# wangruichens/recsys

Hardware: AMD Instinct MI355X
Metric: examples/sec (higher is better)
Workload: dtype f32; 1 GPU; deepfm.py Criteo-39 d=16 DNN 100-100 bs=256/replica, full train step (fwd+bwd+TF1 Adam), adam_mode=tf1_dense, hip_graph=True, steps_per_graph=16; global_batch=256, parallelism=dp1, adam_window=8, reported=median repeat

## Files before the change

include/rsx.h:

```cpp
#ifndef RSX_H_
#define RSX_H_
#include <stddef.h>
#include <stdint.h>

#ifdef __cplusplus
extern "C" {
#endif

typedef void* rsx_stream_t;

typedef enum {
  RSX_OK = 0,
  RSX_EINVAL = -1,
  RSX_ELAUNCH = -2,
  RSX_EUNSUPPORTED = -3,
  RSX_EDATA = -4,
  RSX_ECOMM = -5
} rsx_status;

int rsx_version(void);
unsigned long long rsx_dbg_launch_count(void);
const char* rsx_strerror(int status);


// ... 32 lines not shown
                           float* E, float* S, float* y1, float* y2, uint64_t w1_field_mask, int B, int F, int D,
                           const rsx_sort_job* sort_h, rsx_stream_t stream);

typedef struct {
  const int32_t* segid;
  float* P;
  float* P1;
  float* G;
  float* gw1;
  const int32_t* row_off;
  int32_t null_row;
  uint64_t skip_mask;
} rsx_seg_partials;
#define RSX_NULL_NONE (-1)
#define RSX_NULL_LAST_ROW (-2)
typedef struct {
  int32_t examples;
  int64_t stride_floats;
} rsx_example_blocks;
int rsx_segsum_partials(const float* tables, const float* S, const float* dX, const float* gy1, const float* gy2,
                        const int32_t* perm, const int32_t* seg_off, const int32_t* uniq_row,
                        const rsx_seg_partials* ws_h, uint64_t w1_field_mask, int B, int F, int D, int stride,
                        int null_row, const rsx_example_blocks* blocks_h, rsx_stream_t stream);


int rsx_segsum_bwd(const float* tables, const float* S, const float* dX, const float* gy1, const float* gy2,
                   const int32_t* perm, const int32_t* seg_off, const int32_t* uniq_row, const int32_t* nuniq,
                   float* G, float* gw1, uint64_t w1_field_mask, int B, int F, int D, int stride,
                   const rsx_seg_partials* partials_h, const rsx_example_blocks* blocks_h, rsx_stream_t stream);

typedef enum {
  RSX_ADAM_DENSE = 0,
  RSX_ADAM_TABLE_TF1 = 1,
  RSX_ADAM_VEC_SLOT = 2,
  RSX_ADAM_TABLE_ROWS = 3,
  RSX_ADAM_VEC_ROWS = 4,
  RSX_ADAM_TABLE_TF1_COLD = 5,
  RSX_ADAM_VEC_COLD = 6,
  RSX_ADAM_VEC_ROWS_DENSE = 7
} rsx_adam_kind;

typedef struct {
  int32_t kind;
  int32_t d;
  int64_t n;
  float* var;
  float* m;
  float* v;
  float* g;
  const int32_t* slot;
  const int32_t* uniq_row;
  const int32_t* nuniq;
  int32_t B;
  int32_t stride;
  int32_t zero_grad;
  const int32_t* slot_w[7];
  int32_t g_replicas;
  int64_t g_replica_stride;
} rsx_adam_seg;

#define RSX_ADAM_MAX_SEGS 12
#define RSX_ADAM_STATE_WORDS (4 + 32 * 32)
int rsx_adam_state_init_h(float* state_h , float beta1, float beta2);
int rsx_adam_tf1_multi(const rsx_adam_seg* segs_h, int nseg, float* state, float lr, float beta1,
                       float beta2, float eps, rsx_stream_t stream);

#define RSX_OPT_ADAGRAD 1
#define RSX_OPT_FTRL 2
typedef struct {
  int32_t kind;
  float lr, lr_power, l1, l2, l2_shrinkage;
} rsx_sparse_opt_hp;
int rsx_sparse_opt_multi(const rsx_adam_seg* segs_h, int nseg, float* state, const rsx_sparse_opt_hp* hp,
                         rsx_stream_t stream);

typedef struct {
  const rsx_adam_seg* segs;
  int32_t nseg;
  float lr, beta1, beta2, eps;
  float* state;
  uint32_t blk_lo, blk_hi;
  int32_t window_block_u;
  int32_t alphas_from_state;
} rsx_adam_slice;
int64_t rsx_adam_num_blocks(const rsx_adam_seg* segs_h, int nseg);
int64_t rsx_adam_num_blocks_u(const rsx_adam_seg* segs_h, int nseg, int window_block_u);
typedef struct rsx_table_set {
  float* tables; float* m; float* v;
  const float* dX;
  const rsx_seg_partials* partials;
} rsx_table_set;
#define RSX_ADAM_WINDOW_MAX 8
typedef struct {
  int32_t k;
  int32_t cur;
  int32_t max_unique;
  const int32_t* uniq_row[RSX_ADAM_WINDOW_MAX];
  const int32_t* nuniq[RSX_ADAM_WINDOW_MAX];
  const int32_t* slot[RSX_ADAM_WINDOW_MAX];
} rsx_adam_window;
int rsx_segsum_adam_rows(float* tables, float* m_t, float* v_t, float* w1, float* m_w, float* v_w, const float* S,
                         const float* dX, const float* gy1, const float* gy2, const int32_t* perm, const int32_t* seg_off,
                         const int32_t* uniq_row, const int32_t* nuniq, uint64_t w1_field_mask, int B, int F, int D,
                         int stride, const rsx_adam_seg* extra_segs_h, int n_extra, const rsx_adam_slice* sweep_h,
                         const rsx_seg_partials* partials_h, const rsx_example_blocks* blocks_h,
                         const rsx_table_set* second_h, const rsx_adam_window* win_h, float* state, int advance_step,
                         float lr, float beta1, float beta2, float eps, rsx_stream_t stream);
int rsx_segsum_adam_rows2(float* tables, float* m_t, float* v_t, float* w1, float* m_w, float* v_w, const float* S,
                          const float* dX, const float* gy1, const float* gy2, const int32_t* perm, const int32_t* seg_off,
                          const int32_t* uniq_row, const int32_t* nuniq, uint64_t w1_field_mask, int B, int F, int D,
                          int stride, const rsx_adam_seg* extra_segs_h, int n_extra, const rsx_adam_slice* sweep_h,
                          const rsx_seg_partials* partials_h, const rsx_example_blocks* blocks_h,
                          const rsx_table_set* second_h, const rsx_adam_window* win_h, float* state, int advance_step,
                          float lr, float beta1, float beta2, float eps, int w1_stride, int w1_sparse_formula,
                          rsx_stream_t stream);

#define RSX_UNIQ_MAX_RANKS 8
#define RSX_UNIQ_MAX_PARTS 64
int rsx_segsum_bwd_packed(const float* tables, const float* S, const float* dX, const float* gy1, const float* gy2,
                          const int32_t* perm, const int32_t* seg_off, const int32_t* uniq_row, const int32_t* nuniq,
                          float* G, float* gw1, uint64_t w1_field_mask, int B, int F, int D, int stride, int null_row,
                          const rsx_seg_partials* partials_h, const int32_t* goff, rsx_stream_t stream);
typedef struct {
  const int32_t* uniq_row;
  const int32_t* nuniq;
  int32_t* keys;
} rsx_uniq_pack_job;
int rsx_uniq_pack(const rsx_uniq_pack_job* jobs_h, int njobs, const int32_t* goff, const int32_t* row_off, int F, int stride,
                  int parts, int max_cap , rsx_stream_t stream);
typedef struct {
  int32_t* uniq_row;
  int32_t* nuniq;
  int32_t* slot;
  int32_t* src;
} rsx_uniq_merge_job;
int rsx_uniq_merge(const int32_t* keys, long long rank_stride, int job_stride, const rsx_uniq_merge_job* jobs_h, int njobs,
                   const int32_t* goff, const int32_t* row_off, int32_t* part_counts, int parts, int max_rows_per_field,
                   int max_entries, int F, int N, int stride, rsx_stream_t stream);
int rsx_merged_adam_rows(float* tables, float* m_t, float* v_t, float* w1, float* m_w, float* v_w, const float* G,
                         const float* gw1, long long rank_stride, int N, const int32_t* src, const int32_t* goff,
                         const int32_t* uniq_row, const int32_t* nuniq, uint64_t w1_field_mask, int max_units, int F, int D,
                         int stride, const rsx_adam_seg* extra_segs_h, int n_extra, const rsx_adam_slice* sweep_h,
                         const rsx_table_set* second_h, const rsx_adam_window* win_h, float* state, int advance_step,
                         float lr, float beta1, float beta2, float eps, int w1_stride, int w1_sparse_formula,
                         rsx_stream_t stream);
#define RSX_COMM_UNIQUE_ID_BYTES 128
typedef void* rsx_comm_t;
int rsx_comm_available_h(int* version_out );
const char* rsx_comm_last_error_h(void);
int rsx_comm_unique_id_h(void* id_out );
int rsx_comm_init_h(const void* unique_id, int rank, int world, rsx_comm_t* comm_out);
int rsx_comm_destroy_h(rsx_comm_t comm);
int rsx_comm_rank_world_h(rsx_comm_t comm, int* rank, int* world);
int rsx_all_gather(rsx_comm_t comm, const void* send, void* recv, size_t bytes_per_rank, rsx_stream_t stream);
int rsx_all_reduce_sum_f32(rsx_comm_t comm, const float* send, float* recv, size_t n, rsx_stream_t stream);
int rsx_all_reduce_all_gather(rsx_comm_t comm, float* grad, size_t n, const void* send, void* recv, size_t bytes_per_rank,
                              rsx_stream_t stream);

int rsx_copy_bytes(void* dst, const void* src, size_t nbytes, rsx_stream_t stream);
int rsx_adam_slice_run(const rsx_adam_slice* slice_h, rsx_stream_t stream);
int rsx_adam_fast_math_selftest(unsigned long long* counts, uint32_t seed, int div_iters, int exhaustive_div,
                                rsx_stream_t stream);

#define RSX_TOWER_FIXED_STATS_MIN_B 513
#define RSX_TOWER_FIXED_STATS_DOUBLES(N) (8 * 4 * (((N) + 15) / 16 * 16))
int rsx_tower_fwd_layer(const float* in, const float* W, const float* bias, float* a_out, double* fstat_out,
// ... 531 lines not shown
```

recsys_amd/_lib.py:

```python
import contextlib
import ctypes as C
import gc
import os

_HERE = os.path.dirname(os.path.abspath(__file__))
LIB_PATH = os.environ.get("RSX_LIB_PATH") or os.path.join(_HERE, "librsx.so")

(RSX_ADAM_DENSE, RSX_ADAM_TABLE_TF1, RSX_ADAM_VEC_SLOT, RSX_ADAM_TABLE_ROWS, RSX_ADAM_VEC_ROWS, RSX_ADAM_TABLE_TF1_COLD,
 RSX_ADAM_VEC_COLD, RSX_ADAM_VEC_ROWS_DENSE) = range(8)
RSX_ADAM_MAX_SEGS = 12
RSX_OPT_ADAGRAD, RSX_OPT_FTRL = 1, 2


class RsxError(RuntimeError):
    pass



FORMS = {
    "scatter_riders": ("1", "reductions only the optimizer reads ride in the scatter's stage-A launch (0: launches of their own)"),
    "sort_in_gather": ("0", "deepfm.py: the dedup sort rides in the gather launch instead of the first tower-forward launch"),
    "sort_ride_max": ("2048", "largest global batch whose dedup sort rides in another launch"),
    "din_side_sort": ("1", "din.py: the ids-only branch (sort + sweep) on a side stream of the step's graph"),
    "din_side_sort_dp": ("1", "the same under data parallelism"),
    "din_gather_ride": ("1", "din.py: the history gather rides in the prepare launch"),
    "mlp_reduce_ride": ("1", "din.py: the fused MLP's gradient reduce rides in the pooling backward launch"),
    "mlp_fuse": ("1", "a batch-norm-free tower as ONE launch (csrc/mlp_fused.hip) instead of 2L + 2"),
    "fm_fuse": ("1", "fm.py: forward + head in one launch"),
    "fuse_gather": ("1", "the input_layer lookup rides in the first tower-forward launch"),
    "gather_cross": ("1", "dcn.py: lookup + cross forward as one launch"),
    "cross_ride": ("1", "dcn.py: the cross layers' backward rides in the last tower layer's backward launch (0: a launch of its own)"),
    "win_separate_sorts": ("0", "debugging aid: an optimizer window's k sorts as k launches"),
    "cin_dx_fsplit": ("1", "xdeepfm.py: the first CIN layer's data gradients split their fields over two workgroups per tile"),
    "cin_wide": ("1", "xdeepfm.py --cin_bf16: the wide-tile kernels"),
    "cin_gather_ride": ("1", "xdeepfm.py: the lookup rides in the filter-preparation launch"),
    "cin_dx0_ride": ("1", "xdeepfm.py: the dX0 tile reduce rides in the weight-gradient launch"),
    "xdfm_sort_ride": ("1", "xdeepfm.py: the dedup sort rides in a tower launch"),
    "dp_eager_tail": ("1", "segmented data-parallel graphs: the step's train_op as an eager tail"),
    "dp_prefetch": ("0", "segmented data-parallel graphs: the next step's ids all-gather issued early"),
    "window_stage": ("", "'memcpy': staged windows fetched with hipMemcpyAsync instead of the copy kernel"),
    "window_sets": ("2", "captured instances of a streaming window that take turns"),
    "input_thread": ("0", "the input iterator on a thread of its own"),
    "launch_thread": ("0", "streaming windows issued by a thread of their own"),
    "adam_window_large": ("4", "steps per optimizer window above the small-batch threshold"),
}


def form(name):
    name = name.lower()
    default = FORMS[name][0]
    spec = os.environ.get("RSX_FORMS")
    if spec:
        for item in spec.split(","):
            k, _, v = item.partition("=")
            k = k.strip().lower()
            if k and k not in FORMS:
                raise RsxError("RSX_FORMS: unknown launch form %r (known: %s)" % (k, ", ".join(sorted(FORMS))))
            if k == name:
                return v.strip()
    return default


class AdamSeg(C.Structure):
    _fields_ = [("kind", C.c_int32), ("d", C.c_int32), ("n", C.c_int64),
                ("var", C.c_void_p), ("m", C.c_void_p), ("v", C.c_void_p), ("g", C.c_void_p),
                ("slot", C.c_void_p), ("uniq_row", C.c_void_p), ("nuniq", C.c_void_p),
                ("B", C.c_int32), ("stride", C.c_int32), ("zero_grad", C.c_int32), ("slot_w", C.c_void_p * 7),
                ("g_replicas", C.c_int32), ("g_replica_stride", C.c_int64)]


class AdamSlice(C.Structure):
    _fields_ = [("segs", C.POINTER(AdamSeg)), ("nseg", C.c_int32), ("lr", C.c_float), ("beta1", C.c_float),
                ("beta2", C.c_float), ("eps", C.c_float), ("state", C.c_void_p), ("blk_lo", C.c_uint32),
                ("blk_hi", C.c_uint32), ("window_block_u", C.c_int32), ("alphas_from_state", C.c_int32)]


class ExampleBlocks(C.Structure):
    _fields_ = [("examples", C.c_int32), ("stride_floats", C.c_int64)]


class SegPartials(C.Structure):
    _fields_ = [("segid", C.c_void_p), ("P", C.c_void_p), ("P1", C.c_void_p), ("G", C.c_void_p), ("gw1", C.c_void_p),
                ("row_off", C.c_void_p), ("null_row", C.c_int32), ("skip_mask", C.c_uint64)]

    def __init__(self, segid=None, P=None, P1=None, G=None, gw1=None, row_off=None, null_row=-1, skip_mask=0):
        super().__init__(segid, P, P1, G, gw1, row_off, null_row, skip_mask)


NULL_NONE, NULL_LAST_ROW = -1, -2


class MlpStep(C.Structure):
    _fields_ = [("X", C.c_void_p), ("W", C.c_void_p * 3), ("b", C.c_void_p * 3), ("masks", C.c_void_p * 3),
                ("wout", C.c_void_p), ("bout", C.c_void_p), ("s0", C.c_void_p), ("labels", C.c_void_p),
                ("rng_step", C.c_void_p), ("prob", C.c_void_p), ("dX", C.c_void_p), ("gs0", C.c_void_p),
                ("workspace", C.c_void_p), ("dW", C.c_void_p * 3), ("db", C.c_void_p * 3), ("dwout", C.c_void_p),
                ("dbout", C.c_void_p), ("loss", C.c_void_p), ("seed", C.c_uint32), ("dropout_rate", C.c_float),
                ("loss_scale", C.c_float), ("B", C.c_int32), ("K0", C.c_int32), ("L", C.c_int32), ("widths", C.c_int32 * 3),
                ("defer_reduce", C.c_int32), ("reserved", C.c_int32)]


class MlpReduceJob(C.Structure):
    _fields_ = [("part", C.c_void_p), ("poff", C.c_longlong * 4), ("dW", C.c_void_p * 3), ("db", C.c_void_p * 3),
                ("dwout", C.c_void_p), ("dbout", C.c_void_p), ("loss", C.c_void_p), ("K", C.c_int32 * 3), ("N", C.c_int32 * 3),
                ("e4_end", C.c_uint32 * 3), ("e4_last", C.c_uint32), ("L", C.c_int32), ("nwg", C.c_int32), ("NPo", C.c_int32),
                ("NL", C.c_int32), ("inv_B", C.c_double)]


class DwReduceJob(C.Structure):
    _fields_ = [("partials", C.c_void_p), ("dW", C.c_void_p), ("db", C.c_void_p), ("sb", C.c_int32), ("K", C.c_int32),
                ("N", C.c_int32), ("layout", C.c_int32)]


class CrossReduceJob(C.Structure):
    _fields_ = [("part", C.c_void_p), ("dW", C.c_void_p), ("dB", C.c_void_p), ("dwout", C.c_void_p), ("RT", C.c_int32),
                ("n", C.c_int32), ("L", C.c_int32), ("dim", C.c_int32)]


class TowerBwdExtra(C.Structure):
    _fields_ = [("accumulate_dx", C.c_int32), ("x0", C.c_void_p), ("cW", C.c_void_p), ("cB", C.c_void_p), ("s", C.c_void_p),
                ("gz", C.c_void_p), ("wout", C.c_void_p), ("dX", C.c_void_p), ("dcW", C.c_void_p), ("dcB", C.c_void_p),
                ("dwout", C.c_void_p), ("workspace", C.c_void_p), ("dim", C.c_int32), ("L", C.c_int32),
                ("reduce_out", C.POINTER(CrossReduceJob))]


class VecReduceJob(C.Structure):
    _fields_ = [("part", C.c_void_p), ("out", C.c_void_p), ("G", C.c_int32), ("n", C.c_int32)]


class ScatterRiders(C.Structure):
    _fields_ = [("dw", DwReduceJob * 4), ("n_dw", C.c_int32), ("n_vec", C.c_int32), ("cross", CrossReduceJob),
                ("vec", VecReduceJob * 2)]


class GatherJob(C.Structure):
    _fields_ = [("table", C.c_void_p), ("ids", C.c_void_p), ("out", C.c_void_p), ("n", C.c_int64), ("K", C.c_int32),
                ("ld_out", C.c_int32), ("row_base", C.c_int32), ("ld_table", C.c_int32)]


class TableSet(C.Structure):
    _fields_ = [("tables", C.c_void_p), ("m", C.c_void_p), ("v", C.c_void_p), ("dX", C.c_void_p), ("partials", C.c_void_p)]


class CinDwJob(C.Structure):
    _fields_ = [("Xk", C.c_void_p), ("ws", C.c_void_p), ("dW", C.c_void_p), ("dc", C.c_void_p), ("H", C.c_int32), ("N", C.c_int32),
                ("dc_rows", C.c_int32)]


class GatherTwoJob(C.Structure):
    _fields_ = [("tables1", C.c_void_p), ("w1", C.c_void_p), ("tables2", C.c_void_p), ("row_off", C.c_void_p), ("ids", C.c_void_p),
                ("num_x", C.c_void_p), ("num_w", C.c_void_p), ("E1", C.c_void_p), ("E2", C.c_void_p), ("y1", C.c_void_p),
                ("w1_field_mask", C.c_uint64), ("B", C.c_int32), ("F", C.c_int32), ("D", C.c_int32), ("ND", C.c_int32)]


class UniqPackJob(C.Structure):
    _fields_ = [("uniq_row", C.c_void_p), ("nuniq", C.c_void_p), ("keys", C.c_void_p)]

# ... 295 lines not shown
```

recsys_amd/csrc/adam.hip:

```cpp
#include "adam_device.h"

__global__ __launch_bounds__(ADAM_T) void adam_multi_k(const AdamArgs a) {
  const float b1p = a.state[0], b2p = a.state[1];
  adam_block(a, blockIdx.x);
  __syncthreads();
  if (threadIdx.x == 0 && adam_arrive_last(a.state, a.total_blocks)) {
    a.state[0] = b1p * a.b1;
    a.state[1] = b2p * a.b2;
    reinterpret_cast<uint32_t*>(a.state)[3] += 1u;
  }
}

extern "C" int rsx_adam_state_init_h(float* state_h, float beta1, float beta2) {
  if (!state_h) return RSX_EINVAL;
  state_h[0] = beta1;
  state_h[1] = beta2;
  reinterpret_cast<uint32_t*>(state_h)[2] = 0u;
  reinterpret_cast<uint32_t*>(state_h)[3] = 1u;
  return RSX_OK;
}

extern "C" int rsx_adam_tf1_multi(const rsx_adam_seg* segs_h, int nseg, float* state, float lr, float beta1,
                                  float beta2, float eps, rsx_stream_t stream) {
  AdamArgs a;
  uint32_t blocks = 0;
  const int rc = adam_build_args(segs_h, nseg, state, lr, beta1, beta2, eps, a, &blocks);
  if (rc != RSX_OK) return rc;
  if (blocks == 0) return RSX_OK;
  RSX_LAUNCH(adam_multi_k, dim3(blocks), dim3(ADAM_T), 0, rsx_s(stream), a);
  RSX_CHECK_LAUNCH();
  return RSX_OK;
}

extern "C" int64_t rsx_adam_num_blocks(const rsx_adam_seg* segs_h, int nseg) {
  return rsx_adam_num_blocks_u(segs_h, nseg, 0);
}
extern "C" int64_t rsx_adam_num_blocks_u(const rsx_adam_seg* segs_h, int nseg, int window_block_u) {
  AdamArgs a;
  uint32_t blocks = 0;
  float dummy;
  const int rc = adam_build_args(segs_h, nseg, &dummy, 0.f, 0.f, 0.f, 0.f, a, &blocks, window_block_u);
  return rc != RSX_OK ? (int64_t)rc : (int64_t)blocks;
}

__global__ __launch_bounds__(ADAM_T) void adam_slice_k(const AdamSlice s) { adam_block(s.args, s.blk_lo + blockIdx.x); }

#ifndef RSX_ADAM_WIN_OCC
#define RSX_ADAM_WIN_OCC 3
#endif
template <int NW>
__global__ __launch_bounds__(ADAM_T, RSX_ADAM_WIN_OCC) void adam_window_k(const AdamSlice s) {
  if (blockIdx.x == 0 && threadIdx.x == 0 && s.blk_lo == 0 && !s.args.alpha_src) adam_publish_step_sizes<NW>(s.args);
  adam_window_block<NW>(s.args, s.blk_lo + blockIdx.x);
}
template <int NW>
static void launch_window(const AdamSlice& s, hipStream_t st) {
  RSX_LAUNCH(adam_window_k<NW>, dim3(s.n_blk), dim3(ADAM_T), 0, st, s);
}

extern "C" int rsx_adam_slice_run(const rsx_adam_slice* slice_h, rsx_stream_t stream) {
  AdamSlice s;
  const int rc = adam_build_slice(slice_h, s);
  if (rc != RSX_OK) return rc;
  if (s.n_blk == 0) return RSX_OK;
  if (s.args.win_u != 0) return RSX_EUNSUPPORTED;
  const dim3 grid(s.n_blk), block(ADAM_T);
  switch (s.args.nw) {
    case 0: RSX_LAUNCH(adam_slice_k, grid, block, 0, rsx_s(stream), s); break;
    case 1: launch_window<1>(s, rsx_s(stream)); break;
    case 2: launch_window<2>(s, rsx_s(stream)); break;
    case 3: launch_window<3>(s, rsx_s(stream)); break;
    case 4: launch_window<4>(s, rsx_s(stream)); break;
    case 5: launch_window<5>(s, rsx_s(stream)); break;
    case 6: launch_window<6>(s, rsx_s(stream)); break;
    default: launch_window<7>(s, rsx_s(stream)); break;
  }
  RSX_CHECK_LAUNCH();
  return RSX_OK;
}

namespace {
__device__ __forceinline__ uint32_t st_mix(uint32_t x) {
  x ^= x >> 16; x *= 0x7feb352du; x ^= x >> 15; x *= 0x846ca68bu; x ^= x >> 16;
  return x;
}
__global__ void st_sqrt_k(const uint32_t lo, const uint32_t hi, unsigned long long* bad) {
  const uint32_t n = hi - lo;
  unsigned long long mine = 0;
  for (uint64_t i = ((uint64_t)blockIdx.x * blockDim.x + threadIdx.x) * 2u; i < n; i += (uint64_t)gridDim.x * blockDim.x * 2u) {
    const uint32_t b0 = lo + (uint32_t)i, b1 = i + 1 < n ? b0 + 1 : b0;
    const float x0 = __uint_as_float(b0), x1 = __uint_as_float(b1);
    const rsx_f2 s = rsx_sqrt2_fast((rsx_f2){x0, x1});
    mine += __float_as_uint(s.x) != __float_as_uint(sqrtf(x0));
    mine += b1 != b0 && __float_as_uint(s.y) != __float_as_uint(sqrtf(x1));
  }
  if (mine) atomicAdd(bad, mine);
}
__global__ void st_div_k(const uint32_t seed, const int iters, unsigned long long* bad) {
  uint32_t s = st_mix(seed ^ (blockIdx.x * blockDim.x + threadIdx.x) * 0x9e3779b9u);
  unsigned long long mine = 0;
  for (int it = 0; it < iters; ++it) {
    float n[2], d[2];
    for (int k = 0; k < 2; ++k) {
      s = st_mix(s + 0x632be5abu);
      const uint32_t en = 127 - 94 + s % (94 + 34 + 1);
      s = st_mix(s + 1);
      const uint32_t ed = 127 - 30 + s % (30 + 21 + 1);
      s = st_mix(s + 2);
      uint32_t mn = s & 0x7fffffu;
      const uint32_t sg = s >> 31;
      if ((s >> 23 & 31u) == 0u) mn = (s >> 28) & 1u ? 0x7fffffu : 0u;
      if (en == 127u + 34u) mn = 0u;
      s = st_mix(s + 3);
      uint32_t md = s & 0x7fffffu;
      if ((s >> 23 & 15u) == 0u) md = (s >> 27) & 1u ? 0x7fffffu : 0u;
      if (ed == 127u + 21u) md = 0u;
      n[k] = __uint_as_float((sg << 31) | (en << 23) | mn);
      if ((s >> 28) == 0u) n[k] = 0.f;
      d[k] = __uint_as_float((ed << 23) | md);
    }
    const rsx_f2 q = rsx_div2_fast((rsx_f2){n[0], n[1]}, (rsx_f2){d[0], d[1]});
    mine += __float_as_uint(q.x) != __float_as_uint(n[0] / d[0]);
    mine += __float_as_uint(q.y) != __float_as_uint(n[1] / d[1]);
  }
  if (mine) atomicAdd(bad, mine);
}

__global__ void st_div_all_k(const uint32_t md_lo, unsigned long long* bad) {
  unsigned long long mine = 0;
  const float d = __uint_as_float(0x3f800000u | (md_lo + blockIdx.x));
  for (uint32_t mn = threadIdx.x * 2u; mn < (1u << 23); mn += blockDim.x * 2u) {
    const float n0 = __uint_as_float(0x3f800000u | mn), n1 = __uint_as_float(0x3f800000u | (mn + 1u));
    const rsx_f2 q = rsx_div2_fast((rsx_f2){n0, n1}, (rsx_f2){d, d});
    mine += __float_as_uint(q.x) != __float_as_uint(n0 / d);
    mine += __float_as_uint(q.y) != __float_as_uint(n1 / d);
  }
  if (mine) atomicAdd(bad, mine);
}
}

extern "C" int rsx_adam_fast_math_selftest(unsigned long long* counts, uint32_t seed, int div_iters, int exhaustive_div,
                                           rsx_stream_t stream) {
  if (!counts || div_iters < 0) return RSX_EINVAL;
  hipStream_t st = rsx_s(stream);
  if (hipMemsetAsync(counts, 0, 4 * sizeof(unsigned long long), st) != hipSuccess) return RSX_ELAUNCH;
  RSX_LAUNCH(st_sqrt_k, dim3(4096), dim3(256), 0, st, (127u - 96u) << 23, (127u + 41u) << 23, counts);
  const int grid = 4096, block = 256;
  if (div_iters > 0) RSX_LAUNCH(st_div_k, dim3(grid), dim3(block), 0, st, seed, div_iters, counts + 1);
  const unsigned long long pairs = 2ull * grid * block * (unsigned long long)div_iters;
  if (hipMemcpyAsync(counts + 2, &pairs, sizeof(pairs), hipMemcpyHostToDevice, st) != hipSuccess) return RSX_ELAUNCH;
  if (exhaustive_div) {
    for (uint32_t lo = 0; lo < (1u << 23); lo += (1u << 18)) {
      RSX_LAUNCH(st_div_all_k, dim3(1u << 18), dim3(256), 0, st, lo, counts + 3);
      if (hipStreamSynchronize(st) != hipSuccess) return RSX_ELAUNCH;
    }
  }
  if (hipStreamSynchronize(st) != hipSuccess) return RSX_ELAUNCH;
  RSX_CHECK_LAUNCH();
// ... 3 lines not shown
```

recsys_amd/csrc/adam_device.h:

```cpp
#pragma once
#include "adam_fast.h"
#include "rsx_common.h"

struct SegDev {
  int32_t kind, d;
  long long n;
  float *var, *m, *v, *g;
  const int32_t *slot, *uniq_row, *nuniq;
  int32_t B, stride, zero_grad;
  uint32_t blk_begin;
  int32_t g_rep, g_rep_stride4;
};
constexpr int ADAM_WMAX = RSX_ADAM_WINDOW_MAX - 1;
struct AdamArgs {
  SegDev seg[RSX_ADAM_MAX_SEGS];
  const int32_t* slot_w0;
  long long slot_w_stride;
  int32_t nw;
  int32_t nseg;
  float lr, b1, b2, eps;
  float* state;
  uint32_t total_blocks;
  int32_t win_u, alpha_src;
};
// ... 273 lines not shown
        const int f = (int)(sidx / s.B), j = (int)(sidx - (long long)f * s.B);
        if (j < s.nuniq[f]) {
          const long long sl = (long long)f * s.stride + j;
          const int r = s.uniq_row[sl];
          float g = s.g[sl];
          for (int rr = 1; rr < s.g_rep; ++rr) g += s.g[(long long)rr * 4 * s.g_rep_stride4 + sl];
          if (s.kind == RSX_ADAM_VEC_ROWS_DENSE) adam_dense1(s.var[r], s.m[r], s.v[r], g, h);
          else adam_sparse1(s.var[r], s.m[r], s.v[r], g, true, h);
        }
      }
    }
  }
}

#ifndef RSX_ADAM_WIN_FAST
#define RSX_ADAM_WIN_FAST 1
#endif

__device__ __forceinline__ float rsx_sqrt1_fast(const float x) {
  const float r = __builtin_amdgcn_rsqf(x), g = x * r, hh = r * 0.5f;
  return __builtin_fmaf(__builtin_fmaf(-g, g, x), hh, g);
}
__device__ __forceinline__ float rsx_div1_fast(const float n, const float d) {
  float r = __builtin_amdgcn_rcpf(d);
  r = __builtin_fmaf(__builtin_fmaf(-d, r, 1.f), r, r);
  const float q = n * r;
  return __builtin_fmaf(__builtin_fmaf(-d, q, n), r, q);
}
template <bool DENSE>
__device__ __forceinline__ void adam_zero_grad1(float& var, float& m, float& v, const bool active, const Hp& h) {
  float m1, v1, n;
  if constexpr (DENSE) {
    m1 = m + (0.f - m) * h.omb1;
    v1 = v + (0.f * 0.f - v) * h.omb2;
    n = m1 * h.alpha;
  } else {
    m1 = m * h.b1;
    v1 = v * h.b2;
    n = h.alpha * m1;
  }
  const bool vz = __float_as_uint(v1) == 0u && __float_as_uint(n) == 0u;
  const float d = (vz ? 0.f : rsx_sqrt1_fast(vz ? 1.f : v1)) + h.eps;
  const uint32_t vb = __float_as_uint(v1), nb = __float_as_uint(n), na = nb & 0x7fffffffu, db = __float_as_uint(d);
  constexpr uint32_t V_LO = (127u - 96u) << 23, V_HI = (127u + 41u) << 23;
  constexpr uint32_t D_LO = (127u - 30u) << 23, D_HI = (127u + 21u) << 23;
  constexpr uint32_t N_LO = (127u - 94u) << 23, N_HI = (127u + 34u) << 23;
  const bool ok = (vz || (vb - V_LO) < (V_HI - V_LO)) && (db - D_LO) <= (D_HI - D_LO) &&
                  (nb == 0u || (na - N_LO) <= (N_HI - N_LO));
  if (RSX_ADAM_WIN_FAST && __builtin_amdgcn_ballot_w64(active && !ok) == 0ull) {
    if (active) {
      var = var - rsx_div1_fast(n, d);
      m = m1;
      v = v1;
    }
  } else if (active) {
    if constexpr (DENSE) adam_dense1(var, m, v, 0.f, h);
    else adam_sparse1(var, m, v, 0.f, false, h);
  }
}


__device__ __forceinline__ void adam_zero_grad2(rsx_f2& var, rsx_f2& m, rsx_f2& v, const float alpha, const Hp& h) {
  m = m * h.b1;
  v = v * h.b2;
  const rsx_f2 n = m * alpha;
  const rsx_f2 d = rsx_sqrt2_fast(v) + h.eps;
  var = var - rsx_div2_fast(n, d);
}
__device__ __forceinline__ bool adam_win_guard1(const float var, const float m, const float v, const uint32_t m_lo_bits) {
  const uint32_t vb = __float_as_uint(v), mb = __float_as_uint(m), ma = mb & 0x7fffffffu;
  const uint32_t va = __float_as_uint(var) & 0x7fffffffu;
  constexpr uint32_t V_LO = (127u - 86u) << 23, V_HI = (127u + 40u) << 23, M_HI = (127u + 30u) << 23;
  constexpr uint32_t VAR_LO = (127u - 24u) << 23;
  const bool v_ok = (vb - V_LO) <= (V_HI - V_LO);
  const bool m_mid = (ma - m_lo_bits) <= (M_HI - m_lo_bits);
  const bool m_tiny = ma < m_lo_bits && va >= VAR_LO;
  return !(mb == 0u ? (v_ok || vb == 0u) : (v_ok && (m_mid || m_tiny)));
}
__device__ __forceinline__ bool adam_win_guard4(const float4& var, const float4& m, const float4& v, const uint32_t m_lo_bits) {
  return adam_win_guard1(var.x, m.x, v.x, m_lo_bits) | adam_win_guard1(var.y, m.y, v.y, m_lo_bits) |
         adam_win_guard1(var.z, m.z, v.z, m_lo_bits) | adam_win_guard1(var.w, m.w, v.w, m_lo_bits);
}

template <int NW, int U = ADAM_U>
__device__ __forceinline__ void adam_window_block(const AdamArgs& a, const uint32_t blk, const int tid = threadIdx.x) {
  constexpr int nw = NW;
  constexpr int HB = RSX_ADAM_WIN_HB;
  constexpr int NB = U / HB;
  static_assert(U % HB == 0 && U <= ADAM_U, "U");
  int si = 0;
#pragma unroll 1
  for (int k = 1; k < a.nseg; ++k)
    if (blk >= a.seg[k].blk_begin) si = k;
  const SegDev& s = a.seg[si];
  if (s.kind != RSX_ADAM_TABLE_TF1_COLD) {
    adam_block(a, blk, tid);
    return;
  }
  Hp h;
  h.b1 = a.b1;
  h.b2 = a.b2;
  h.omb1 = 1.0f - a.b1;
  h.omb2 = 1.0f - a.b2;
  h.eps = a.eps;
  AlphaW aw;
  adam_step_sizes(a, nw, h.alpha, aw);
  float amin = h.alpha, amax = h.alpha;
#pragma unroll
  for (int j = 0; j < NW; ++j) {
    amin = fminf(amin, aw.get(j));
    amax = fmaxf(amax, aw.get(j));
  }
  const bool fast_ok = RSX_ADAM_WIN_FAST && a.b1 >= 0.85f && a.b1 < 1.f && a.b2 >= 0.5f && a.b2 < 1.f && a.eps >= 0x1p-30f &&
                       a.eps <= 1.f && amin >= 0x1p-24f && amax <= 16.f && amax <= 4.f * amin;
  const uint32_t m_lo_bits = __float_as_uint(fast_ok ? 0x1p-90f / amin : 1.f);
  const int32_t* __restrict__ swb = a.slot_w0;
  const int sws = (int)a.slot_w_stride;
  float4* __restrict__ var4 = reinterpret_cast<float4*>(s.var);
  float4* __restrict__ m4 = reinterpret_cast<float4*>(s.m);
  float4* __restrict__ v4 = reinterpret_cast<float4*>(s.v);
  const long long base = (long long)(blk - s.blk_begin) * ((long long)ADAM_T * U);
  const int lpr = s.d >> 2;
  const long long n4 = s.n * lpr;
  const bool pow2 = (lpr & (lpr - 1)) == 0;
  const int lsh = 31 - __clz(lpr);
  struct Batch {
    float4 var[HB], m[HB], v[HB];
    long long ec[HB];
    int t[HB];
    bool live[HB];
  };
  auto issue = [&](const int b, Batch& B) {
#pragma unroll
    for (int u = 0; u < HB; ++u) {
      const long long e = base + (long long)(b * HB + u) * ADAM_T + tid;
      B.ec[u] = e < n4 ? e : n4 - 1;
      B.live[u] = e < n4;
      const long long row = pow2 ? (B.ec[u] >> lsh) : (B.ec[u] / lpr);
      B.t[u] = s.slot[row];
#pragma unroll
      for (int l = 0; l < NW; ++l) B.t[u] &= swb[l * sws + (int)row];
    }
#pragma unroll
    for (int u = 0; u < HB; ++u) {
#if RSX_ADAM_NT
      B.var[u] = __builtin_nontemporal_load(&var4[B.ec[u]]);
      B.m[u] = __builtin_nontemporal_load(&m4[B.ec[u]]);
      B.v[u] = __builtin_nontemporal_load(&v4[B.ec[u]]);
#else
      B.var[u] = var4[B.ec[u]];
      B.m[u] = m4[B.ec[u]];
      B.v[u] = v4[B.ec[u]];
#endif
    }
  };
  auto store = [&](const Batch& B) {
#pragma unroll
    for (int u = 0; u < HB; ++u) {
      if (B.live[u] && B.t[u] < 0) {
#if RSX_ADAM_NT
        __builtin_nontemporal_store(B.var[u], &var4[B.ec[u]]);
        __builtin_nontemporal_store(B.m[u], &m4[B.ec[u]]);
        __builtin_nontemporal_store(B.v[u], &v4[B.ec[u]]);
#else
        var4[B.ec[u]] = B.var[u];
        m4[B.ec[u]] = B.m[u];
        v4[B.ec[u]] = B.v[u];
#endif
      }
    }
  };
  uint32_t redo = fast_ok ? 0u : (1u << NB) - 1u;
  auto finish = [&](const int b, Batch& B) {
    if (!fast_ok) return;
    bool bad = false;
#pragma unroll
    for (int u = 0; u < HB; ++u) bad |= adam_win_guard4(B.var[u], B.m[u], B.v[u], m_lo_bits);
    if (__builtin_amdgcn_ballot_w64(bad) != 0ull) {
      redo |= 1u << b;
      return;
    }
    rsx_f2 var2[HB][2], m2[HB][2], v2[HB][2];
#pragma unroll
    for (int u = 0; u < HB; ++u) {
      var2[u][0] = (rsx_f2){B.var[u].x, B.var[u].y}; var2[u][1] = (rsx_f2){B.var[u].z, B.var[u].w};
      m2[u][0] = (rsx_f2){B.m[u].x, B.m[u].y}; m2[u][1] = (rsx_f2){B.m[u].z, B.m[u].w};
      v2[u][0] = (rsx_f2){B.v[u].x == 0.f ? 1.f : B.v[u].x, B.v[u].y == 0.f ? 1.f : B.v[u].y};
      v2[u][1] = (rsx_f2){B.v[u].z == 0.f ? 1.f : B.v[u].z, B.v[u].w == 0.f ? 1.f : B.v[u].w};
    }
    auto step = [&](const float alpha) {
#pragma unroll
      for (int u = 0; u < HB; ++u) {
        adam_zero_grad2(var2[u][0], m2[u][0], v2[u][0], alpha, h);
        adam_zero_grad2(var2[u][1], m2[u][1], v2[u][1], alpha, h);
      }
    };
    step(h.alpha);
#pragma unroll 1
    for (int j = 0; j < NW; ++j) step(aw.get(j));
#pragma unroll
    for (int u = 0; u < HB; ++u) {
      B.var[u] = make_float4(var2[u][0].x, var2[u][0].y, var2[u][1].x, var2[u][1].y);
      B.m[u] = make_float4(m2[u][0].x, m2[u][0].y, m2[u][1].x, m2[u][1].y);
      B.v[u] = make_float4(B.v[u].x == 0.f ? 0.f : v2[u][0].x, B.v[u].y == 0.f ? 0.f : v2[u][0].y,
                           B.v[u].z == 0.f ? 0.f : v2[u][1].x, B.v[u].w == 0.f ? 0.f : v2[u][1].y);
    }
    store(B);
  };
  {
    Batch bt[2];
    issue(0, bt[0]);
#pragma unroll
    for (int b = 0; b < NB; ++b) {
      if (b + 1 < NB) issue(b + 1, bt[(b + 1) & 1]);
      finish(b, bt[b & 1]);
    }
  }
  redo = __builtin_amdgcn_readfirstlane(redo);
  if (redo != 0u) {
#pragma unroll 1
    for (int b = 0; b < NB; ++b) {
      if (!(redo >> b & 1u)) continue;
      Batch B;
      issue(b, B);
#pragma unroll
      for (int u = 0; u < HB; ++u) {
        F4_APPLY(adam_sparse1, B.var[u], B.m[u], B.v[u], F4Z, false, h);
#pragma unroll 1
        for (int j = 0; j < NW; ++j) {
          Hp hj = h;
          hj.alpha = aw.get(j);
          F4_APPLY(adam_sparse1, B.var[u], B.m[u], B.v[u], F4Z, false, hj);
        }
      }
      store(B);
    }
  }
}

static inline int adam_build_args(const rsx_adam_seg* segs_h, int nseg, float* state, float lr, float beta1, float beta2,
                                  float eps, AdamArgs& a, uint32_t* blocks_out, int win_u = 0, int alpha_src = 0) {
  if (!segs_h || !state || nseg <= 0 || nseg > RSX_ADAM_MAX_SEGS) return RSX_EINVAL;
  if (win_u != 0 && win_u != 2 && win_u != 4 && win_u != ADAM_U) return RSX_EINVAL;
  a.win_u = win_u == ADAM_U ? 0 : win_u;
  a.alpha_src = alpha_src ? 1 : 0;
  uint32_t blocks = 0;
  int k = 0, n_cold = 0;
  a.nw = 0;
  a.slot_w0 = nullptr;
  a.slot_w_stride = 0;
  for (int i = 0; i < nseg; ++i) {
    const rsx_adam_seg& s = segs_h[i];
    if (s.n < 0 || !s.var || !s.m || !s.v) return RSX_EINVAL;
    long long work;
    switch (s.kind) {
      case RSX_ADAM_DENSE:
        if (!s.g) return RSX_EINVAL;
        if (s.B > 1 && (s.stride < s.n || (s.stride & 3))) return RSX_EINVAL;
        work = (s.n >> 2) + 1;
        break;
      case RSX_ADAM_TABLE_TF1:
      case RSX_ADAM_TABLE_TF1_COLD:
        if (!s.slot || (!s.g && s.kind == RSX_ADAM_TABLE_TF1) || s.d < 4 || (s.d & 3)) return RSX_EINVAL;
        if (s.kind == RSX_ADAM_TABLE_TF1 && s.slot_w[0]) return RSX_EINVAL;
        work = s.n * (s.d >> 2);
        break;
      case RSX_ADAM_VEC_SLOT:
      case RSX_ADAM_VEC_COLD:
        if (!s.slot || (!s.g && s.kind == RSX_ADAM_VEC_SLOT)) return RSX_EINVAL;
        if (s.kind == RSX_ADAM_VEC_SLOT && s.slot_w[0]) return RSX_EINVAL;
        work = (s.n >> 2) + 1;
        break;
      case RSX_ADAM_TABLE_ROWS:
        if (!s.g || !s.uniq_row || !s.nuniq || s.B <= 0 || s.d < 4 || (s.d & 3)) return RSX_EINVAL;
        if (s.g_replicas > 1 && (s.g_replica_stride <= 0 || (s.g_replica_stride & 3) || s.g_replica_stride >= (1ll << 33))) return RSX_EINVAL;
        work = s.n * (s.d >> 2);
        break;
      case RSX_ADAM_VEC_ROWS:
      case RSX_ADAM_VEC_ROWS_DENSE:
        if (!s.g || !s.uniq_row || !s.nuniq || s.B <= 0) return RSX_EINVAL;
        if (s.g_replicas > 1 && (s.g_replica_stride <= 0 || (s.g_replica_stride & 3) || s.g_replica_stride >= (1ll << 33))) return RSX_EINVAL;
        work = s.n;
        break;
      default: return RSX_EINVAL;
    }
    if (s.n == 0) continue;
    SegDev& d = a.seg[k++];
    d.kind = s.kind;
    d.d = s.d;
    d.n = s.n;
    d.var = s.var;
    d.m = s.m;
    d.v = s.v;
    d.g = s.g;
    d.slot = s.slot;
    d.uniq_row = s.uniq_row;
    d.nuniq = s.nuniq;
    d.B = s.B;
    d.stride = s.stride;
    d.zero_grad = s.zero_grad;
    const bool rows_kind = s.kind == RSX_ADAM_TABLE_ROWS || s.kind == RSX_ADAM_VEC_ROWS || s.kind == RSX_ADAM_VEC_ROWS_DENSE;
    d.g_rep = rows_kind && s.g_replicas > 1 ? s.g_replicas : 1;
    d.g_rep_stride4 = d.g_rep > 1 ? (int32_t)(s.g_replica_stride >> 2) : 0;
    if (s.kind == RSX_ADAM_TABLE_TF1_COLD || s.kind == RSX_ADAM_VEC_COLD) {
      int nw = 0;
      while (nw < ADAM_WMAX && s.slot_w[nw] != nullptr) ++nw;
      for (int j = nw; j < ADAM_WMAX; ++j)
// ... 60 lines not shown
```

recsys_amd/ops.py:

```python
import ctypes as C
import os

import numpy as np
import torch

from . import _lib
from ._lib import AdamSeg, check, lib


def _ptr(t):
    return None if t is None else C.c_void_p(t.data_ptr())


def _stream():
    return C.c_void_p(torch.cuda.current_stream().cuda_stream)


def make_scatter_riders(dw_jobs=None, cross_job=None, vec_jobs=None):
    dw_jobs = list(dw_jobs or ())
    vec_jobs = [v for v in (vec_jobs or ()) if v.n > 0]
    if not dw_jobs and (cross_job is None or cross_job.n == 0) and not vec_jobs:
        return None
    r = _lib.ScatterRiders()
    if len(dw_jobs) > len(r.dw) or len(vec_jobs) > len(r.vec):
# ... 507 lines not shown
    def __getitem__(self, k):
        return self.params[k]

    def load(self, values):
        with torch.no_grad():
            for k, v in values.items():
                if k in self.params:
                    self.params[k].copy_(torch.as_tensor(np.asarray(v), dtype=torch.float32).reshape(self.params[k].shape))

    def adam_segments(self):
        return [dict(kind=_lib.RSX_ADAM_DENSE, n=self.n, var=self.flat, m=self.m, v=self.v, g=self.grad,
                     zero_grad=1)]

    def rebind_grad(self, storage):
        assert storage.is_contiguous() and storage.numel() >= self.n and storage.dtype == torch.float32
        g = storage[:self.n]
        g.copy_(self.grad)
        self.grad = g
        for k, p in self.params.items():
            st = self.storage[k]
            sz = int(np.prod(st)) if len(st) else 1
            o = self.offsets[k]
            p.grad = g[o:o + sz].view(st)[tuple(slice(0, d) for d in p.shape)]

    def packed_grad(self, names):
        o = self.offsets[names[0]]
        e = o
        for k in names:
            if self.offsets[k] != e or tuple(self.params[k].shape) != self.storage[k]:
                return None
            e += self.params[k].numel()
        return self.grad[o:e]


class AdamTF1:

    def __init__(self, lr=1e-3, beta1=0.9, beta2=0.999, eps=1e-8, device="cuda"):
        dev = _require_cuda(device)
        self.hp = (float(lr), float(beta1), float(beta2), float(eps))
        st = np.zeros(_lib.ADAM_STATE_WORDS, np.float32)
        check(lib().rsx_adam_state_init_h(st.ctypes.data_as(C.c_void_p), beta1, beta2))
        self.state = torch.from_numpy(st).to(dev)

    @staticmethod
    def _seg_array(segments):
        n = len(segments)
        arr = (AdamSeg * n)()
        for i, s in enumerate(segments):
            a = arr[i]
            a.kind, a.d, a.n = s["kind"], s.get("d", 0), int(s["n"])
            for f in ("var", "m", "v", "g", "slot", "uniq_row", "nuniq"):
                t = s.get(f)
                setattr(a, f, None if t is None else t.data_ptr())
            a.B, a.stride, a.zero_grad = s.get("B", 0), s.get("stride", 0), s.get("zero_grad", 0)
            a.g_replicas, a.g_replica_stride = int(s.get("g_replicas", 0)), int(s.get("g_replica_stride", 0))
            for j, t in enumerate(s.get("slot_w") or ()):
                a.slot_w[j] = t.data_ptr()
        return arr, n

    def step(self, segments):
        arr, n = self._seg_array(segments)
        lr, b1, b2, eps = self.hp
        check(lib().rsx_adam_tf1_multi(arr, n, _ptr(self.state), lr, b1, b2, eps, _stream()), "rsx_adam_tf1_multi")

    def cold_slices(self, cold_segments, weights, window_block_u=0):
        if getattr(self, "shadow", False):
            return [None] * len(weights)
        arr, n = self._seg_array(cold_segments)
        nb = int(lib().rsx_adam_num_blocks_u(arr, n, int(window_block_u)))
        if nb < 0:
            check(nb, "rsx_adam_num_blocks")
        lr, b1, b2, eps = self.hp
        tot = float(sum(weights))
        out, lo, acc = [], 0, 0.0
        for i, w in enumerate(weights):
            acc += w
            hi = nb if i == len(weights) - 1 else min(nb, int(round(nb * acc / tot)))
            if hi > lo:
                sl = _lib.AdamSlice()
                sl.segs, sl.nseg, sl.lr, sl.beta1, sl.beta2, sl.eps = arr, n, lr, b1, b2, eps
                sl.state, sl.blk_lo, sl.blk_hi = self.state.data_ptr(), lo, hi
                sl.window_block_u = int(window_block_u)
                sl.alphas_from_state = 1 if (window_block_u and lo > 0) else 0
                sl._keep = arr
                out.append(sl)
            else:
                out.append(None)
            lo = hi
        return out

    def run_slice(self, sl):
        if sl is None:
            return
        check(lib().rsx_adam_slice_run(C.byref(sl), _stream()), "rsx_adam_slice_run")

    def window_sweep(self, cold_segments):
        self.run_slice(self.cold_slices(cold_segments, [1.0])[0])

    @property
    def global_step(self):
        return int(self.state.view(torch.int32)[3].item()) - 1


class _SparseOptTF1:
    name = None
    KIND = None

    def __init__(self, lr, initial_accumulator_value, device, lr_power=-0.5, l1=0.0, l2=0.0, l2_shrinkage=0.0):
        self.hparams = self._check(lr, initial_accumulator_value, lr_power, l1, l2, l2_shrinkage)
        dev = _require_cuda(device)
        self.initial_accumulator_value = float(initial_accumulator_value)
        self.hp = _lib.SparseOptHp(self.KIND, float(lr), float(lr_power), float(l1), float(l2), float(l2_shrinkage))
        st = np.zeros(_lib.ADAM_STATE_WORDS, np.float32)
        st.view(np.uint32)[3] = 1
        self.state = torch.from_numpy(st).to(dev)

    @staticmethod
    def _check(lr, acc0, lr_power, l1, l2, l2_shrinkage):
        raise NotImplementedError

    def step(self, segments):
        arr, n = AdamTF1._seg_array(segments)
        check(lib().rsx_sparse_opt_multi(arr, n, _ptr(self.state), C.byref(self.hp), _stream()), "rsx_sparse_opt_multi")

    @property
    def global_step(self):
        return int(self.state.view(torch.int32)[3].item()) - 1


class AdagradTF1(_SparseOptTF1):
    name = "adagrad"
    KIND = _lib.RSX_OPT_ADAGRAD

    def __init__(self, lr=1e-3, initial_accumulator_value=0.1, device="cuda"):
        super().__init__(lr, initial_accumulator_value, device)

    @staticmethod
    def _check(lr, acc0, lr_power, l1, l2, l2_shrinkage):
        if not float(lr) > 0.0:
            raise ValueError("AdagradOptimizer: learning_rate must be > 0, got %r" % (lr,))
        if not float(acc0) > 0.0:
            raise ValueError("AdagradOptimizer: initial_accumulator_value must be > 0, got %r" % (acc0,))
        return {"learning_rate": float(lr), "initial_accumulator_value": float(acc0)}


class FtrlTF1(_SparseOptTF1):
    name = "ftrl"
    KIND = _lib.RSX_OPT_FTRL

    def __init__(self, lr=1e-3, learning_rate_power=-0.5, initial_accumulator_value=0.1, l1_regularization_strength=0.0,
                 l2_regularization_strength=0.0, l2_shrinkage_regularization_strength=0.0, device="cuda"):
        super().__init__(lr, initial_accumulator_value, device, learning_rate_power, l1_regularization_strength,
                         l2_regularization_strength, l2_shrinkage_regularization_strength)

    @staticmethod
    def _check(lr, acc0, lr_power, l1, l2, l2_shrinkage):
        if not float(lr) > 0.0:
            raise ValueError("FtrlOptimizer: learning_rate must be > 0, got %r" % (lr,))
        if not float(lr_power) <= 0.0:
            raise ValueError("FtrlOptimizer: learning_rate_power must be <= 0, got %r" % (lr_power,))
        if not float(acc0) >= 0.0:
            raise ValueError("FtrlOptimizer: initial_accumulator_value must be >= 0, got %r" % (acc0,))
        for k, v in (("l1_regularization_strength", l1), ("l2_regularization_strength", l2),
                     ("l2_shrinkage_regularization_strength", l2_shrinkage)):
            if not float(v) >= 0.0:
                raise ValueError("FtrlOptimizer: %s must be >= 0, got %r" % (k, v))
# ... 771 lines not shown
```

Measured before the change: 4.592 million examples/sec.

## Compact Adam window sweep to rows with nonzero moments before applying updates

Adds a compact path to the windowed cold-table Adam sweep. A first pass reads only m and v, votes per row across the wave, and handles rows whose first moment is zero by scaling v in place. Indices of rows that still need the full Adam update go into an LDS list, and a second pass runs Adam only on those. This is meant to cut var loads and update arithmetic for the many untouched rows in large embedding tables. The cost is an extra classification pass, LDS use and a block barrier, with a fallback to the dense pass when a wave is mostly live.

```diff
diff --git a/include/rsx.h b/include/rsx.h
--- a/include/rsx.h
+++ b/include/rsx.h
@@ -138,6 +138,7 @@
   uint32_t blk_lo, blk_hi;
   int32_t window_block_u;
   int32_t alphas_from_state;
+  int32_t window_compact;
 } rsx_adam_slice;
 int64_t rsx_adam_num_blocks(const rsx_adam_seg* segs_h, int nseg);
 int64_t rsx_adam_num_blocks_u(const rsx_adam_seg* segs_h, int nseg, int window_block_u);
diff --git a/recsys_amd/_lib.py b/recsys_amd/_lib.py
--- a/recsys_amd/_lib.py
+++ b/recsys_amd/_lib.py
@@ -43,6 +43,7 @@
     "input_thread": ("0", "the input iterator on a thread of its own"),
     "launch_thread": ("0", "streaming windows issued by a thread of their own"),
     "adam_window_large": ("4", "steps per optimizer window above the small-batch threshold"),
+    "window_compact": ("1", "the window sweep classifies rows first and runs Adam only on rows with moments (0: one pass over all)"),
 }
 
 
@@ -72,7 +73,8 @@
 class AdamSlice(C.Structure):
     _fields_ = [("segs", C.POINTER(AdamSeg)), ("nseg", C.c_int32), ("lr", C.c_float), ("beta1", C.c_float),
                 ("beta2", C.c_float), ("eps", C.c_float), ("state", C.c_void_p), ("blk_lo", C.c_uint32),
-                ("blk_hi", C.c_uint32), ("window_block_u", C.c_int32), ("alphas_from_state", C.c_int32)]
+                ("blk_hi", C.c_uint32), ("window_block_u", C.c_int32), ("alphas_from_state", C.c_int32),
+                ("window_compact", C.c_int32)]
 
 
 class ExampleBlocks(C.Structure):
diff --git a/recsys_amd/csrc/adam.hip b/recsys_amd/csrc/adam.hip
--- a/recsys_amd/csrc/adam.hip
+++ b/recsys_amd/csrc/adam.hip
@@ -48,14 +48,20 @@
 #ifndef RSX_ADAM_WIN_OCC
 #define RSX_ADAM_WIN_OCC 3
 #endif
-template <int NW>
+template <int NW, bool COMPACT>
 __global__ __launch_bounds__(ADAM_T, RSX_ADAM_WIN_OCC) void adam_window_k(const AdamSlice s) {
   if (blockIdx.x == 0 && threadIdx.x == 0 && s.blk_lo == 0 && !s.args.alpha_src) adam_publish_step_sizes<NW>(s.args);
-  adam_window_block<NW>(s.args, s.blk_lo + blockIdx.x);
+  if constexpr (COMPACT) {
+    __shared__ uint32_t lds[WIN_LIST_WORDS];
+    adam_window_block<NW, ADAM_U, true>(s.args, s.blk_lo + blockIdx.x, threadIdx.x, lds);
+  } else {
+    adam_window_block<NW>(s.args, s.blk_lo + blockIdx.x);
+  }
 }
 template <int NW>
-static void launch_window(const AdamSlice& s, hipStream_t st) {
-  RSX_LAUNCH(adam_window_k<NW>, dim3(s.n_blk), dim3(ADAM_T), 0, st, s);
+static void launch_window(const AdamSlice& s, const bool compact, hipStream_t st) {
+  if (compact) RSX_LAUNCH((adam_window_k<NW, true>), dim3(s.n_blk), dim3(ADAM_T), 0, st, s);
+  else RSX_LAUNCH((adam_window_k<NW, false>), dim3(s.n_blk), dim3(ADAM_T), 0, st, s);
 }
 
 extern "C" int rsx_adam_slice_run(const rsx_adam_slice* slice_h, rsx_stream_t stream) {
@@ -64,16 +70,22 @@
   if (rc != RSX_OK) return rc;
   if (s.n_blk == 0) return RSX_OK;
   if (s.args.win_u != 0) return RSX_EUNSUPPORTED;
+  bool compact = slice_h->window_compact != 0;
+  for (int k = 0; k < s.args.nseg; ++k) {
+    const int lpr = s.args.seg[k].d >> 2;
+    if (s.args.seg[k].kind == RSX_ADAM_TABLE_TF1_COLD && (lpr > 64 || (lpr & (lpr - 1)) != 0)) compact = false;
+  }
   const dim3 grid(s.n_blk), block(ADAM_T);
+  hipStream_t st = rsx_s(stream);
   switch (s.args.nw) {
-    case 0: RSX_LAUNCH(adam_slice_k, grid, block, 0, rsx_s(stream), s); break;
-    case 1: launch_window<1>(s, rsx_s(stream)); break;
-    case 2: launch_window<2>(s, rsx_s(stream)); break;
-    case 3: launch_window<3>(s, rsx_s(stream)); break;
-    case 4: launch_window<4>(s, rsx_s(stream)); break;
-    case 5: launch_window<5>(s, rsx_s(stream)); break;
-    case 6: launch_window<6>(s, rsx_s(stream)); break;
-    default: launch_window<7>(s, rsx_s(stream)); break;
+    case 0: RSX_LAUNCH(adam_slice_k, grid, block, 0, st, s); break;
+    case 1: launch_window<1>(s, compact, st); break;
+    case 2: launch_window<2>(s, compact, st); break;
+    case 3: launch_window<3>(s, compact, st); break;
+    case 4: launch_window<4>(s, compact, st); break;
+    case 5: launch_window<5>(s, compact, st); break;
+    case 6: launch_window<6>(s, compact, st); break;
+    default: launch_window<7>(s, compact, st); break;
   }
   RSX_CHECK_LAUNCH();
   return RSX_OK;
diff --git a/recsys_amd/csrc/adam_device.h b/recsys_amd/csrc/adam_device.h
--- a/recsys_amd/csrc/adam_device.h
+++ b/recsys_amd/csrc/adam_device.h
@@ -379,12 +379,23 @@
          adam_win_guard1(var.z, m.z, v.z, m_lo_bits) | adam_win_guard1(var.w, m.w, v.w, m_lo_bits);
 }
 
-template <int NW, int U = ADAM_U>
-__device__ __forceinline__ void adam_window_block(const AdamArgs& a, const uint32_t blk, const int tid = threadIdx.x) {
+constexpr int WIN_LIST_WORDS = ADAM_T * ADAM_U + 1;
+template <int NW>
+__device__ __forceinline__ bool win_shortcut_gate(const AdamArgs& a, const float alpha0, const AlphaW& aw) {
+  auto plus_finite = [](const float x) { return __float_as_uint(x) < 0x7f800000u; };
+  bool ok = plus_finite(a.eps) && a.eps > 0.f && plus_finite(a.b1) && plus_finite(a.b2) && a.b2 > 0.f && plus_finite(alpha0);
+#pragma unroll
+  for (int j = 0; j < NW; ++j) ok = ok && plus_finite(aw.get(j));
+  return ok;
+}
+template <int NW, int U = ADAM_U, bool COMPACT = false>
+__device__ __forceinline__ void adam_window_block(const AdamArgs& a, const uint32_t blk, const int tid = threadIdx.x,
+                                                  uint32_t* const lds = nullptr ) {
   constexpr int nw = NW;
   constexpr int HB = RSX_ADAM_WIN_HB;
   constexpr int NB = U / HB;
   static_assert(U % HB == 0 && U <= ADAM_U, "U");
+  static_assert(!COMPACT || (U == ADAM_U && ADAM_T % 64 == 0), "the compact form: full-size blocks of whole waves");
   int si = 0;
 #pragma unroll 1
   for (int k = 1; k < a.nseg; ++k)
@@ -427,7 +438,21 @@
     int t[HB];
     bool live[HB];
   };
-  auto issue = [&](const int b, Batch& B) {
+  auto load_state = [&](Batch& B, const bool with_var) {
+#pragma unroll
+    for (int u = 0; u < HB; ++u) {
+#if RSX_ADAM_NT
+      if (with_var) B.var[u] = __builtin_nontemporal_load(&var4[B.ec[u]]);
+      B.m[u] = __builtin_nontemporal_load(&m4[B.ec[u]]);
+      B.v[u] = __builtin_nontemporal_load(&v4[B.ec[u]]);
+#else
+      if (with_var) B.var[u] = var4[B.ec[u]];
+      B.m[u] = m4[B.ec[u]];
+      B.v[u] = v4[B.ec[u]];
+#endif
+    }
+  };
+  auto issue = [&](const int b, Batch& B, const bool with_var = true) {
 #pragma unroll
     for (int u = 0; u < HB; ++u) {
       const long long e = base + (long long)(b * HB + u) * ADAM_T + tid;
@@ -438,18 +463,7 @@
 #pragma unroll
       for (int l = 0; l < NW; ++l) B.t[u] &= swb[l * sws + (int)row];
     }
-#pragma unroll
-    for (int u = 0; u < HB; ++u) {
-#if RSX_ADAM_NT
-      B.var[u] = __builtin_nontemporal_load(&var4[B.ec[u]]);
-      B.m[u] = __builtin_nontemporal_load(&m4[B.ec[u]]);
-      B.v[u] = __builtin_nontemporal_load(&v4[B.ec[u]]);
-#else
-      B.var[u] = var4[B.ec[u]];
-      B.m[u] = m4[B.ec[u]];
-      B.v[u] = v4[B.ec[u]];
-#endif
-    }
+    load_state(B, with_var);
   };
   auto store = [&](const Batch& B) {
 #pragma unroll
@@ -467,10 +481,9 @@
       }
     }
   };
-  uint32_t redo = fast_ok ? 0u : (1u << NB) - 1u;
+  uint32_t redo = 0u;
   auto finish = [&](const int b, Batch& B) {
-    if (!fast_ok) return;
-    bool bad = false;
+    bool bad = !fast_ok;
 #pragma unroll
     for (int u = 0; u < HB; ++u) bad |= adam_win_guard4(B.var[u], B.m[u], B.v[u], m_lo_bits);
     if (__builtin_amdgcn_ballot_w64(bad) != 0ull) {
@@ -504,7 +517,122 @@
     }
     store(B);
   };
-  {
+  const int lane = tid & 63;
+  const uint32_t wave_first = (((uint32_t)__builtin_amdgcn_readfirstlane(tid >> 6) + blk) % (ADAM_T / 64u)) * (64u * HB);
+  uint32_t n_live = 0u;
+  auto listed = [&](const int b) { return (uint32_t)b * (ADAM_T * HB) + wave_first < n_live; };
+  auto issue_listed = [&](const int b, Batch& B) {
+#pragma unroll
+    for (int u = 0; u < HB; ++u) {
+      const uint32_t idx = (uint32_t)b * (ADAM_T * HB) + wave_first + (uint32_t)u * 64u + (uint32_t)lane;
+      B.live[u] = idx < n_live;
+      B.ec[u] = base + (B.live[u] ? lds[idx] : 0u);
+      B.t[u] = -1;
+    }
+    load_state(B, true);
+  };
+  if constexpr (COMPACT) {
+    const bool gate = win_shortcut_gate<NW>(a, h.alpha, aw);
+    const unsigned long long row_lanes = (lpr >= 64 ? ~0ull : (1ull << lpr) - 1ull) << (lane & ~(lpr - 1));
+    uint32_t* const list_n = lds + ADAM_T * U;
+    if (tid == 0) *list_n = 0u;
+    __syncthreads();
+    auto vote = [&](const Batch& B, const int u, bool& untouched, bool& still, bool& row_v0) {
+      const uint32_t mx = __float_as_uint(B.m[u].x), my = __float_as_uint(B.m[u].y), mz = __float_as_uint(B.m[u].z),
+                     mw = __float_as_uint(B.m[u].w);
+      const uint32_t vx = __float_as_uint(B.v[u].x), vy = __float_as_uint(B.v[u].y), vz = __float_as_uint(B.v[u].z),
+                     vw = __float_as_uint(B.v[u].w);
+      const uint32_t v_top = max(max(vx, vy), max(vz, vw));
+      const bool row_m0 = (__builtin_amdgcn_ballot_w64((mx | my | mz | mw) != 0u) & row_lanes) == 0ull;
+      const bool row_vok = (__builtin_amdgcn_ballot_w64(v_top > 0x7f800000u) & row_lanes) == 0ull;
+      row_v0 = (__builtin_amdgcn_ballot_w64((vx | vy | vz | vw) != 0u) & row_lanes) == 0ull;
+      untouched = B.live[u] && B.t[u] < 0;
+      still = gate && row_m0 && row_vok;
+    };
+    auto wave_dense = [&](const Batch& B) {
+      unsigned long long due = 0ull, spared = 0ull;
+#pragma unroll
+      for (int u = 0; u < HB; ++u) {
+        bool untouched, still, row_v0;
+        vote(B, u, untouched, still, row_v0);
+        due |= __builtin_amdgcn_ballot_w64(untouched);
+        spared |= __builtin_amdgcn_ballot_w64(untouched && still);
+      }
+      return !gate || (due != 0ull && spared == 0ull);
+    };
+    auto classify = [&](const Batch& B) {
+      unsigned long long lm[HB];
+      bool is_live[HB];
+      uint32_t total = 0u;
+#pragma unroll
+      for (int u = 0; u < HB; ++u) {
+        bool untouched, still, row_v0;
+        vote(B, u, untouched, still, row_v0);
+        is_live[u] = untouched && !still;
+        lm[u] = __builtin_amdgcn_ballot_w64(is_live[u]);
+        total += (uint32_t)__popcll(lm[u]);
+        if (untouched && still && !row_v0) {
+          float4 v = B.v[u];
+#pragma unroll
+          for (int j = 0; j < 1 + NW; ++j) {
+            v.x = v.x * h.b2;
+            v.y = v.y * h.b2;
+            v.z = v.z * h.b2;
+            v.w = v.w * h.b2;
+          }
+#if RSX_ADAM_NT
+          __builtin_nontemporal_store(v, &v4[B.ec[u]]);
+#else
+          v4[B.ec[u]] = v;
+#endif
+        }
+      }
+      if (total != 0u) {
+        uint32_t at = 0u;
+        if (lane == 0) at = atomicAdd(list_n, total);
+        at = (uint32_t)__builtin_amdgcn_readfirstlane((int)at);
+#pragma unroll
+        for (int u = 0; u < HB; ++u) {
+          const uint32_t before = __builtin_amdgcn_mbcnt_hi((uint32_t)(lm[u] >> 32), __builtin_amdgcn_mbcnt_lo((uint32_t)lm[u], 0u));
+          if (is_live[u]) lds[at + before] = (uint32_t)(B.ec[u] - base);
+          at += (uint32_t)__popcll(lm[u]);
+        }
+      }
+    };
+    bool dense;
+    {
+      Batch bt[2];
+      issue(0, bt[0], false);
+      dense = wave_dense(bt[0]);
+      if (!dense) {
+#pragma unroll
+        for (int b = 0; b < NB; ++b) {
+          if (b + 1 < NB) issue(b + 1, bt[(b + 1) & 1], false);
+          classify(bt[b & 1]);
+        }
+      }
+    }
+    __syncthreads();
+    n_live = (uint32_t)__builtin_amdgcn_readfirstlane((int)*list_n);
+    {
+      Batch bt[2];
+      if (listed(0)) issue_listed(0, bt[0]);
+#pragma unroll
+      for (int b = 0; b < NB; ++b) {
+        if (b + 1 < NB && listed(b + 1)) issue_listed(b + 1, bt[(b + 1) & 1]);
+        if (listed(b)) finish(NB + b, bt[b & 1]);
+      }
+    }
+    if (dense) {
+      Batch bt[2];
+      issue(0, bt[0]);
+#pragma unroll
+      for (int b = 0; b < NB; ++b) {
+        if (b + 1 < NB) issue(b + 1, bt[(b + 1) & 1]);
+        finish(b, bt[b & 1]);
+      }
+    }
+  } else {
     Batch bt[2];
     issue(0, bt[0]);
 #pragma unroll
@@ -516,10 +644,11 @@
   redo = __builtin_amdgcn_readfirstlane(redo);
   if (redo != 0u) {
 #pragma unroll 1
-    for (int b = 0; b < NB; ++b) {
+    for (int b = 0; b < (COMPACT ? 2 * NB : NB); ++b) {
       if (!(redo >> b & 1u)) continue;
       Batch B;
-      issue(b, B);
+      if (COMPACT && b >= NB) issue_listed(b - NB, B);
+      else issue(b, B);
 #pragma unroll
       for (int u = 0; u < HB; ++u) {
         F4_APPLY(adam_sparse1, B.var[u], B.m[u], B.v[u], F4Z, false, h);
diff --git a/recsys_amd/ops.py b/recsys_amd/ops.py
--- a/recsys_amd/ops.py
+++ b/recsys_amd/ops.py
@@ -613,6 +613,7 @@
                 sl.state, sl.blk_lo, sl.blk_hi = self.state.data_ptr(), lo, hi
                 sl.window_block_u = int(window_block_u)
                 sl.alphas_from_state = 1 if (window_block_u and lo > 0) else 0
+                sl.window_compact = 0 if window_block_u else int(_lib.form("window_compact") != "0")
                 sl._keep = arr
                 out.append(sl)
             else:
```

New measurement: 4.754 million examples/sec, median of 6. +3.5%, better.
